# duburcqa/jiminy

Hardware: AMD Instinct MI355X
Metric: env-steps/s (whole node) ANYmal 18-DoF batch 65536; achieved HBM GB/s vs peak (higher is better)
Workload: dtype f64

## Files before the change

jiminy_amd/csrc/jm_quad.h:

```cpp
#pragma once
#include "jm_kernels.h"

namespace jm
{
template<class Tp> struct QLayout
{
    static constexpr int J_PLC = 0, J_RBI = 12, J_AXIS = 22, J_AXP = 25, J_ROTOR = 28, J_QLO = 29, J_QHI = 30, J_MOTOR = 31, J_ENC = 40;
    static constexpr int QJ = 41;
    static constexpr int C_IDX = 12, C_CS = 13, C_FREL = 14;
    static constexpr int QC = Tp::QHAS_FORCE ? 26 : 14;
    static constexpr int CONTACT = Tp::QN * QJ;
    static constexpr int RAW = CONTACT + Tp::QCL * QC;
    static constexpr int QSTRIDE = (RAW % 2 == 0) ? RAW + 1 : RAW;
    static constexpr int TABLE = 4 * QSTRIDE;
    static constexpr int OFFSET = Layout<Tp>::TOTAL;
    static constexpr int TOTAL = OFFSET + TABLE;
};

JM_DEV int sel4(int k, int c0, int c1, int c2, int c3) { return k == 0 ? c0 : (k == 1 ? c1 : (k == 2 ? c2 : c3)); }

template<class Tp> struct QInfo
{
    static constexpr int N = Tp::QN, NT = Tp::QT;
    static constexpr int NQB = 7 + (NT - 1), NVB = 6 + (NT - 1);
    static constexpr bool limb_at(int t)
    {
        for (int k = 0; k < 4; ++k) if (Tp::limb_attach[k] == t) return true;
        return false;
    }
    static constexpr bool child_after(int t, int c)
    {
        for (int i = c + 1; i < NT; ++i) if (Tp::trunk_parent[i] == t) return true;
        return false;
    }
    static constexpr bool has_child(int t) { return limb_at(t) || child_after(t, t); }
    static constexpr bool first_contrib(int c) { return !limb_at(Tp::trunk_parent[c]) && !child_after(Tp::trunk_parent[c], c); }
    static constexpr bool uniform_attach = Tp::limb_attach[0] == Tp::limb_attach[1] && Tp::limb_attach[0] == Tp::limb_attach[2] && Tp::limb_attach[0] == Tp::limb_attach[3];
    static constexpr int qrow(int i) { return i < 7 ? Tp::idx_q[1] + i : Tp::idx_q[Tp::trunk_joint[i - 6]]; }
    static constexpr int vrow(int i) { return i < 6 ? Tp::idx_v[1] + i : Tp::idx_v[Tp::trunk_joint[i - 5]]; }
};

template<class Tp> constexpr int limb_axis_uniform(int s)
{
    int ax = -2;
    for (int k = 0; k < 4; ++k)
    {
        const int c = s < Tp::limb_len[k] ? Tp::axis_signed[Tp::limb_joint[k][s]] : 1;
        if (c == 0) return -1;
        const int a = (c < 0 ? -c : c) - 1;
        if (ax == -2) ax = a;
        else if (ax != a) return -1;
    }
    return ax;
}
template<class Tp> constexpr bool limb_axis_negative(int s)
{
    for (int k = 0; k < 4; ++k)
        if (s < Tp::limb_len[k] && Tp::axis_signed[Tp::limb_joint[k][s]] < 0) return true;
    return false;
}
template<class T> JM_DEV V3<T> mcol(const M3<T> & R, int ax)
{
    return ax == 0 ? V3<T>{R.m00, R.m10, R.m20} : (ax == 1 ? V3<T>{R.m01, R.m11, R.m21} : V3<T>{R.m02, R.m12, R.m22});
}
template<class T> JM_DEV M3<T> mul_rot_axis(const M3<T> & R, int ax, T c, T s)
{
    if (ax == 0) return {R.m00, c * R.m01 + s * R.m02, c * R.m02 - s * R.m01, R.m10, c * R.m11 + s * R.m12, c * R.m12 - s * R.m11,
                         R.m20, c * R.m21 + s * R.m22, c * R.m22 - s * R.m21};
    if (ax == 1) return {c * R.m00 - s * R.m02, R.m01, c * R.m02 + s * R.m00, c * R.m10 - s * R.m12, R.m11, c * R.m12 + s * R.m10,
                         c * R.m20 - s * R.m22, R.m21, c * R.m22 + s * R.m20};
    return {c * R.m00 + s * R.m01, c * R.m01 - s * R.m00, R.m02, c * R.m10 + s * R.m11, c * R.m11 - s * R.m10, R.m12,
            c * R.m20 + s * R.m21, c * R.m21 - s * R.m20, R.m22};
}
template<class T> struct LimbTable
{
    const T * base;
    JM_DEV T operator()(int off) const { return base[off]; }
    JM_DEV V3<T> v3(int o) const { return {base[o], base[o + 1], base[o + 2]}; }
    JM_DEV M3<T> m3(int o) const { return {base[o], base[o + 1], base[o + 2], base[o + 3], base[o + 4], base[o + 5], base[o + 6], base[o + 7], base[o + 8]}; }
    JM_DEV SE3<T> se3(int o) const { return {m3(o), v3(o + 9)}; }
    JM_DEV RBI<T> rbi(int o) const { return {base[o], v3(o + 1), S3<T>{base[o + 4], base[o + 5], base[o + 6], base[o + 7], base[o + 8], base[o + 9]}}; }
};
template<class T, class Tp, int s> JM_DEV V3<T> limb_axis_root(const LimbTable<T> & LT, const M3<T> & Rs_)
{
// ... 456 lines not shown
    {
        a = R * LT.v3(o + Q::J_AXP);
        R = R * (plc.R * rot_rodrigues(LT.v3(o + Q::J_AXIS), c, sn));
    }
}
template<class T, class Tp, int s, class MA = NoModelLane>
JM_DEV void limb_unwind(const LimbTable<T> & LT, T c, T sn, M3<T> & R, V3<T> & p, const MA & ma = MA{}, int k = 0)
{
    using Q = QLayout<Tp>;
    constexpr int o = s * Q::QJ;
    SE3<T> plc = LT.se3(o + Q::J_PLC);
    if constexpr (!std::is_same<MA, NoModelLane>::value)
        plc.p = ma.plc_p(sel4(k, Tp::limb_joint[0][s], Tp::limb_joint[1][s], Tp::limb_joint[2][s], Tp::limb_joint[3][s]), plc.p);
    constexpr int ax = limb_axis_uniform<Tp>(s);
    M3<T> Rq;
    if constexpr (ax >= 0) Rq = mul_rot_axis(R, ax, c, -sn);
    else Rq = R * rot_rodrigues(LT.v3(o + Q::J_AXIS), c, -sn);
    R = mul_bt(Rq, plc.R);
    p = p - R * plc.p;
}

template<class T> JM_DEV Sp<T> applied_wrench_on(const BatchArgs<T> & A, int jq, const M3<T> & R1, const M3<T> & Rj, V3<T> pj,
                                                 unsigned B32, unsigned r32, T te)
{
    Sp<T> f = zero6<T>();
    for (int i = 0; i < A.applied_k; ++i)
    {
        if (A.applied_joint[i] != jq) continue;
        V3<T> F = zero3<T>(), M = zero3<T>();
        if (A.applied)
        {
            const unsigned o = (unsigned)(6 * i) * B32 + r32;
            F = {A.applied[o], A.applied[o + B32], A.applied[o + 2 * B32]};
            M = {A.applied[o + 3 * B32], A.applied[o + 4 * B32], A.applied[o + 5 * B32]};
        }
        if (A.proc_off > 0) add_process_forces(A, i, te, (long long)B32, (long long)r32, F, M);
        const V3<T> p = pj + Rj * V3<T>{A.applied_p[3 * i], A.applied_p[3 * i + 1], A.applied_p[3 * i + 2]};
        const V3<T> fl = tmul(R1, F);
        f.l = f.l + fl;
        f.a = f.a + tmul(R1, M) + cross(p, fl);
    }
    return f;
}
template<class T> JM_DEV Sp<T> applied_root_wrench(const BatchArgs<T> & A, const M3<T> & R1, unsigned B32, unsigned r32, T te)
{
    return applied_wrench_on(A, 1, R1, ident3<T>(), zero3<T>(), B32, r32, te);
}
template<class T> JM_DEV Sp<T> wrench_to_joint(const M3<T> & Rj, V3<T> pj, Sp<T> w)
{
    return {tmul(Rj, w.l), tmul(Rj, w.a - cross(pj, w.l))};
}

template<class T, class Tp> struct QExtra
{
    T tau_l[Tp::QN], tau_b[Tp::QT], uemit_l[Tp::QN], uemit_b[Tp::QT];
    bool motors_on;
    const int32_t * flags;
    const T * lam;
    int nb;
};
struct NoKeep { static constexpr bool ON = false; };
template<class T, class Tp> struct TrunkStore;
template<class T, class Tp> struct QKeep
{
    static constexpr bool ON = true;
    V3<T> ps[Tp::QN], as[Tp::QN];
    Sp<T> Us[Tp::QN];
    T dinv[Tp::QN];
    M3<T> Rt;
    Sp<T> vtip, atip;
    M3<T> R1; V3<T> p1;
    Sp<T> agf1;
    T rootL[6][6], rootdinv[6];
};

template<class T, class Tp, class X, bool EMIT, class SB, int CFM = 0, class KEEP = NoKeep, bool GEN = false, bool DYN = true>
JM_DEV void quad_eval(CPtr<T> P, const LimbTable<T> & LT, const BatchArgs<T> & A, unsigned r, int k, const QIdx<Tp> & ix,
                      const SB & S_, const T * qb, const T * vb_, const T * ql, const T * vl_,
                      bool sensors, T * ddqb, T * ddq, int & status, const QExtra<T, Tp> * ex = nullptr, KEEP * keep = nullptr,
                      TrunkStore<T, Tp> * ts_out = nullptr, T te = T(0))
{
    (void)te;
    using RW = QRows<Tp>;
    auto vlq = [&](int s) -> T { if constexpr (RW::LONG) return S_.getl(RW::KVL + s); else return vl_[s]; };
    auto vbq = [&](int i) -> T { if constexpr (RW::LONG) return S_.getb(RW::KVB + i); else return vb_[i]; };
    auto cmdlq = [&](int s) -> T { return S_.getl(RW::CMDL + s); };
    auto cmdbq = [&](int t) -> T { return S_.getb(RW::CMDB + t); };
    constexpr bool emit = EMIT;
    using L = Layout<Tp>;
    using Q = QLayout<Tp>;
    using I = QInfo<Tp>;
    constexpr int N = Tp::QN, NT = Tp::QT;
    constexpr int FL = Tp::motor_flags[0];
    const unsigned B32 = (unsigned)A.B;
    unsigned r32 = r;
    JM_OPAQUE(r32);
    unsigned Bg = B32, rg = r32;
    if constexpr (GEN)
        if (A.lane_map) { rg = (unsigned)A.lane_map[r32]; Bg = (unsigned)A.B_full; }
    const bool lead = (k == 0);
    const bool emit_sens = emit && sensors;
    const bool want_energy = emit && A.energy;
    if constexpr (Tp::QHAS_ENC)
        if (emit_sens && A.encoder)
        {
            static_for<0, N>([&](auto sc) {
                constexpr int s = decltype(sc)::value;
                const int si = sel4(k, Tp::limb_enc[0][s], Tp::limb_enc[1][s], Tp::limb_enc[2][s], Tp::limb_enc[3][s]);
                T pos = ql[s], vel = vlq(s);
                if constexpr (Tp::QENC_SIDE == 0)
                {
                    const T red = LT(s * Q::QJ + Q::J_ENC);
                    pos *= red;
                    vel *= red;
                }
                if (ix.has[s])
                {
                    A.encoder[(unsigned)(2 * si) * B32 + r32] = pos;
                    A.encoder[(unsigned)(2 * si + 1) * B32 + r32] = vel;
                }
            });
            if (lead)
                static_for<1, NT>([&](auto tc) {
                    constexpr int t = decltype(tc)::value;
                    constexpr int si = Tp::trunk_enc[t];
                    T pos = qb[6 + t], vel = vbq(5 + t);
                    if constexpr (Tp::QENC_SIDE == 0) { pos *= P[L::ENC + si]; vel *= P[L::ENC + si]; }
                    A.encoder[(unsigned)(2 * si) * B32 + r32] = pos;
                    A.encoder[(unsigned)(2 * si + 1) * B32 + r32] = vel;
                });
        }
    const M3<T> R1 = quat_to_matrix(qb[3], qb[4], qb[5], qb[6]);
    const V3<T> p1 = {qb[0], qb[1], qb[2]};
    V3<T> p1g = p1;
    if constexpr (GEN)
        if (A.ground_off) { p1g.x += A.ground_off[rg]; p1g.y += A.ground_off[Bg + rg]; }
    const V3<T> g = ld_v3<T>(P, L::OPT), gw = ld_v3<T>(P, L::OPT + 3);
    const Sp<T> v1 = {{vb_[0], vb_[1], vb_[2]}, {vb_[3], vb_[4], vb_[5]}};
    const Sp<T> agf1 = actinv_motion(SE3<T>{R1, p1}, Sp<T>{-g, -gw});
    TrunkStore<T, Tp> TS;
#ifdef JM_HOST_EMU
    std::memset(&TS, 0xFF, sizeof(TS));
#endif
    SE3<T> Xatt;
    Sp<T> vatt;
    using MA = std::conditional_t<GEN, ModelLane<T>, NoModelLane>;
    MA ma;
    if constexpr (GEN) ma = ModelLane<T>{A.model_lane, Bg, rg};
    auto limb_joint_of = [&](auto sc) {
        constexpr int s = decltype(sc)::value;
        return sel4(k, Tp::limb_joint[0][s], Tp::limb_joint[1][s], Tp::limb_joint[2][s], Tp::limb_joint[3][s]);
    };
    (void)limb_joint_of;
    trunk_fk_store<T, Tp, X, MA>(P, k, ix, qb, vb_, TS, Xatt, vatt, status, ma);
    constexpr bool UNWIND = QRows<Tp>::LONG || !DYN;
    constexpr bool REWIND = UNWIND;
    M3<T> Rs[UNWIND ? 1 : N];
    V3<T> ps[N];
    T cq[UNWIND ? N : 1], sq[UNWIND ? N : 1];
    M3<T> Rtip;
    V3<T> ptip;
    Sp<T> vtip;
    if constexpr (UNWIND) limb_fk_tip<T, Tp, MA>(LT, Xatt, vatt, ql, vl_, cq, sq, Rtip, ptip, vtip, status, ma, k);
    else
    {
        limb_fk<T, Tp, MA>(LT, ix, Xatt, vatt, ql, vl_, Rs, ps, vtip, status, ma, k);
        Rtip = Rs[N - 1]; ptip = ps[N - 1];
    }
// ... 367 lines not shown
                        const Sp<T> vf = actinv_motion(fr, vj);
                        Sp<T> af = actinv_motion(fr, aj);
                        af.l = af.l + cross(vf.a, vf.l);
                        const V3<T> acc3 = af.l - tmul(fr.R, gj);
                        put6(A.imu, B32, r32, 6 * s, Sp<T>{vf.a, acc3});
                    }
                });
    };
    imu_at(std::integral_constant<int, 0>{}, SE3<T>{ident3<T>(), zero3<T>()}, v1r, at0);
    Sp<T> ap = at0;
    Sp<T> vp = v1r;
    M3<T> Rw = ident3<T>();
    V3<T> pw = zero3<T>();
    Sp<T> atst[TrunkStore<T, Tp>::SLOTS];
    {
        Sp<T> aprev = at0;
        static_for<1, NT>([&](auto tc) {
            constexpr int t = decltype(tc)::value;
            constexpr int tp = Tp::trunk_parent[t];
            SE3<T> Xt;
            Sp<T> vt, Ut;
            T di, uj;
            TS.template get_kin<t, X>(Xt, vt);
            if constexpr (DYN) TS.template get_aba<t, X>(Ut, di, uj);
            const Sp<T> S = trunk_S_at<T, Tp, t>(P, Xt);
            const Sp<T> vj = vbq(5 + t) * S;
            Sp<T> apar;
            if constexpr (tp == 0) apar = at0;
            else if constexpr (tp == t - 1) apar = aprev;
            else apar = qbcast<T, X, TrunkStore<T, Tp>::template lane<tp>()>(atst[TrunkStore<T, Tp>::template slot<tp>()]);
            const Sp<T> ag = apar + cross_mm(vt - vj, vj);
            T dd;
            if constexpr (DYN) { dd = di * (uj - dot6(Ut, ag)); ddqb[5 + t] = dd; }
            else dd = ddqb[5 + t];
            const Sp<T> att = ag + dd * S;
            if (TrunkStore<T, Tp>::template first_fwd<t>() || k == TrunkStore<T, Tp>::template lane<t>())
                atst[TrunkStore<T, Tp>::template slot<t>()] = att;
            aprev = att;
            if constexpr (I::limb_at(t))
                if (ix.attach == t)
                {
                    ap = att; vp = vt;
                    if constexpr (REWIND) { Rw = Xt.R; pw = Xt.p; }
                }
            imu_at(tc, Xt, vt, att);
        });
    }
    if constexpr (DYN)
    static_for<0, N>([&](auto sc) {
        constexpr int s = decltype(sc)::value;
        if constexpr (KEEP_SC)
        {
            const Sp<T> ag = ap + cs[s];
            const T dd = ix.has[s] ? dinv[s] * (u[s] - dot6(Us[s], ag)) : T(0);
            ddq[s] = dd;
            ap = ag + dd * Ss[s];
        }
        else
        {
            V3<T> a_s, p_s;
            if constexpr (REWIND)
            {
                limb_rewind<T, Tp, s, MA>(LT, cq[s], sq[s], Rw, pw, a_s, ma, k);
                p_s = pw;
            }
            else { a_s = as[s]; p_s = ps[s]; }
            const Sp<T> S = {cross(p_s, a_s), a_s};
            const Sp<T> vj = vlq(s) * S;
            const Sp<T> ag = ap + cross_mm(vp, vj);
            const T dd = ix.has[s] ? dinv[s] * (u[s] - dot6(Us[s], ag)) : T(0);
            ddq[s] = dd;
            ap = ag + dd * S;
            vp = vp + vj;
        }
    });
    if constexpr (!DYN && EMIT)
    {
        bool applied_out = false;
        if constexpr (GEN) applied_out = A.applied_k > 0 && A.f_external;
        const bool want_rnea = A.joint_forces || A.centroidal;
        if (want_energy || want_rnea || applied_out)
        {
            const bool has_gw = gw.x != T(0) || gw.y != T(0) || gw.z != T(0);
            Sp<T> acur = ap;
            {
                Sp<T> vrun = vp;
                static_for<0, N>([&](auto sc) {
                    constexpr int s = decltype(sc)::value;
                    V3<T> a_s, p_s;
                    if constexpr (REWIND)
                    {
                        limb_rewind<T, Tp, s, MA>(LT, cq[s], sq[s], Rw, pw, a_s, ma, k);
                        p_s = pw;
                    }
                    else { a_s = limb_axis_root<T, Tp, s>(LT, Rs[s]); p_s = ps[s]; }
                    const Sp<T> S = {cross(p_s, a_s), a_s};
                    const Sp<T> vj = vlq(s) * S;
                    acur = acur + cross_mm(vrun, vj) + ddq[s] * S;
                    vrun = vrun + vj;
                });
            }
            Sp<T> hs = zero6<T>(), fjs = zero6<T>(), fxs = fext, Gs = zero6<T>();
            T ms = T(0), ekin = T(0), erot = T(0);
            V3<T> mcs = zero3<T>();
            {
                Sp<T> vcur = vtip;
                M3<T> Rcur = Rtip;
                V3<T> pcur = ptip;
                static_rfor<0, N>([&](auto sc) {
                    constexpr int s = decltype(sc)::value;
                    constexpr int o = s * Q::QJ;
                    if constexpr (!UNWIND) { Rcur = Rs[s]; pcur = ps[s]; }
                    const RBI<T> Y = rbi_placed(Rcur, pcur, ma.rbi(GEN ? limb_joint_of(sc) : 0, LT.rbi(o + Q::J_RBI)));
                    const V3<T> a = limb_axis_root<T, Tp, s>(LT, Rcur);
                    const Sp<T> S = {cross(pcur, a), a};
                    const Sp<T> h = rbi_mul(Y, vcur);
                    hs = hs + h;
                    fjs = fjs + cross_mf(vcur, h) + rbi_mul(Y, acur);
                    if (has_gw) Gs = Gs + rbi_mul(Y, agf1);
                    if constexpr (s == N - 1) fjs = fjs - fext;
                    if constexpr (GEN)
                        if (A.applied_k > 0)
                        {
                            const Sp<T> w = applied_wrench_on(A, limb_joint_of(sc), R1, Rcur, pcur, Bg, rg, te);
                            fjs = fjs - w;
                            fxs = fxs + w;
                            if (applied_out && ix.has[s]) add6(A.f_external, B32, r32, 6u * (unsigned)limb_joint_of(sc), wrench_to_joint(Rcur, pcur, w));
                        }
                    ms += Y.m;
                    mcs = mcs + Y.m * Y.c;
                    ekin += dot6(vcur, h);
                    erot += LT(o + Q::J_ROTOR) * vlq(s) * vlq(s);
                    if (A.joint_forces && ix.has[s])
                        put6(A.joint_forces, B32, r32, 6 * (unsigned)limb_joint_of(sc), actinv_force(SE3<T>{Rcur, pcur}, fjs));
                    const Sp<T> vj = vlq(s) * S;
                    vcur = vcur - vj;
                    acur = acur - cross_mm(vcur, vj) - ddq[s] * S;
                    if constexpr (UNWIND && s > 0) limb_unwind<T, Tp, s, MA>(LT, cq[s], sq[s], Rcur, pcur, ma, k);
                });
            }
            Sp<T> htot = quad_sum6<T, X>(hs), fxtot = quad_sum6<T, X>(fxs), Gtot = zero6<T>();
            if (has_gw) Gtot = quad_sum6<T, X>(Gs);
            T mtot = X::quad_sum(ms);
            V3<T> mctot = {X::quad_sum(mcs.x), X::quad_sum(mcs.y), X::quad_sum(mcs.z)};
            ekin = X::quad_sum(ekin); erot = X::quad_sum(erot);
            Sp<T> fjT[NT];
            static_for<0, NT>([&](auto tc) {
                constexpr int t = decltype(tc)::value;
                if constexpr (I::limb_at(t))
                {
                    if constexpr (I::uniform_attach) fjT[t] = quad_sum6<T, X>(fjs);
                    else fjT[t] = quad_sum6<T, X>(mask6(ix.attach == t, fjs));
                }
                else fjT[t] = zero6<T>();
            });
            static_rfor<0, NT>([&](auto tc) {
                constexpr int t = decltype(tc)::value;
                constexpr int j = Tp::trunk_joint[t];
                SE3<T> Xt = {ident3<T>(), zero3<T>()};
                Sp<T> vt = v1r, att = at0;
                RBI<T> Y = ma.rbi(j, ld_rbi<T>(P, L::JOINT + j * L::JSTRIDE + 12));
                if constexpr (t > 0)
                {
                    TS.template get_kin<t, X>(Xt, vt);
                    att = qbcast<T, X, TrunkStore<T, Tp>::template lane<t>()>(atst[TrunkStore<T, Tp>::template slot<t>()]);
                    Y = rbi_placed(Xt.R, Xt.p, Y);
                }
                const Sp<T> h = rbi_mul(Y, vt);
                htot = htot + h;
                fjT[t] = fjT[t] + cross_mf(vt, h) + rbi_mul(Y, att);
                if (has_gw) Gtot = Gtot + rbi_mul(Y, agf1);
                if constexpr (GEN)
                    if (A.applied_k > 0)
                    {
                        Sp<T> w;
                        if constexpr (t == 0) w = applied_root_wrench(A, R1, Bg, rg, te);
                        else
                        {
                            w = applied_wrench_on(A, j, R1, Xt.R, Xt.p, Bg, rg, te);
                            if (applied_out && lead) put6(A.f_external, B32, r32, 6 * j, wrench_to_joint(Xt.R, Xt.p, w));
                        }
                        fjT[t] = fjT[t] - w;
                        fxtot = fxtot + w;
                    }
                mtot += Y.m;
                mctot = mctot + Y.m * Y.c;
                ekin += dot6(vt, h);
                if constexpr (t > 0) erot += P[L::ROTOR + Tp::idx_v[j]] * vbq(5 + t) * vbq(5 + t);
                if (A.joint_forces && lead)
                {
                    if constexpr (t > 0) put6(A.joint_forces, B32, r32, 6 * j, actinv_force(Xt, fjT[t]));
                    else put6(A.joint_forces, B32, r32, 6 * j, fjT[t]);
                }
                if constexpr (t > 0) fjT[Tp::trunk_parent[t]] = fjT[Tp::trunk_parent[t]] + fjT[t];
            });
            if (lead)
            {
                if (A.joint_forces) put6(A.joint_forces, B32, r32, 0, zero6<T>());
                if (want_energy)
                {
#pragma unroll
                    for (int i = 0; i < 6; ++i) erot += P[L::ROTOR + Tp::idx_v[1] + i] * vb_[i] * vb_[i];
                    A.energy[r32] = T(0.5) * ekin + T(0.5) * erot;
                    A.energy[B32 + r32] = -(dot(R1 * mctot, g) + mtot * dot(p1, g));
                }
                if (A.centroidal)
                {
                    if (!has_gw) Gtot = {mtot * agf1.l, cross(mctot, agf1.l)};
                    const Sp<T> fBtot = fjT[0] + fxtot - Gtot;
                    const SE3<T> M1 = {R1, p1};
                    const V3<T> c1 = rcp_(mtot) * mctot;
                    const V3<T> com0 = R1 * c1 + p1;
                    Sp<T> hg = act_force(M1, htot), dhg = act_force(M1, fBtot);
                    hg.a = hg.a + cross(hg.l, com0);
                    dhg.a = dhg.a + cross(dhg.l, com0);
                    A.centroidal[r32] = com0.x; A.centroidal[B32 + r32] = com0.y; A.centroidal[2 * B32 + r32] = com0.z;
                    put6(A.centroidal, B32, r32, 3, hg);
                    put6(A.centroidal, B32, r32, 9, dhg);
                }
            }
        }
    }
    if constexpr (KEEP::ON)
    {
        keep->atip = ap;
        if (ts_out) *ts_out = TS;
    }
    if constexpr (DYN)
    {
        bool bad = false;
        static_for<0, I::NVB>([&](auto ic) { bad |= (ddqb[decltype(ic)::value] != ddqb[decltype(ic)::value]); });
        static_for<0, N>([&](auto sc) { bad |= ix.has[decltype(sc)::value] && (ddq[decltype(sc)::value] != ddq[decltype(sc)::value]); });
        if (bad) status |= JM_LANE_NAN;
    }
}

template<class T, class Tp, class X, int CFM = 0, bool GEN = false>
JM_DEV void quad_extra_terms(CPtr<T> P, const LimbTable<T> & LT, const BatchArgs<T> & A, unsigned r32, int k, const QIdx<Tp> & ix,
                             const T * qb, const T * vb, const T * ql, const T * vl, const T * ddqb, const T * ddq,
                             const QExtra<T, Tp> * ex = nullptr, T te = T(0))
{
    (void)te;
    using L = Layout<Tp>;
    using Q = QLayout<Tp>;
    using I = QInfo<Tp>;
    constexpr int N = Tp::QN, NT = Tp::QT;
    const unsigned B32 = (unsigned)A.B;
    unsigned Bg = B32, rg = r32;
    if constexpr (GEN)
        if (A.lane_map) { rg = (unsigned)A.lane_map[r32]; Bg = (unsigned)A.B_full; }
    const bool lead = (k == 0);
    const V3<T> g = ld_v3<T>(P, L::OPT), gw = ld_v3<T>(P, L::OPT + 3);
    const M3<T> R1 = quat_to_matrix(qb[3], qb[4], qb[5], qb[6]);
    const V3<T> p1 = {qb[0], qb[1], qb[2]};
    const SE3<T> M1 = {R1, p1};
    V3<T> p1g = p1;
    if constexpr (GEN)
        if (A.ground_off) { p1g.x += A.ground_off[rg]; p1g.y += A.ground_off[Bg + rg]; }
    const Sp<T> agf1 = actinv_motion(M1, Sp<T>{-g, -gw});
    int status = 0;
    using MA = std::conditional_t<GEN, ModelLane<T>, NoModelLane>;
    MA ma;
    if constexpr (GEN) ma = ModelLane<T>{A.model_lane, Bg, rg};
    TrunkKin<T, Tp> K;
    trunk_fk<T, Tp, MA>(P, qb, vb, K, status, ma);
    Sp<T> at[NT];
    at[0] = {{ddqb[0], ddqb[1], ddqb[2]}, {ddqb[3], ddqb[4], ddqb[5]}};
    static_for<1, NT>([&](auto tc) {
        constexpr int t = decltype(tc)::value;
        const Sp<T> S = trunk_S<T, Tp, t>(P, K);
        at[t] = at[Tp::trunk_parent[t]] + cross_mm(K.v[t], vb[5 + t] * S) + ddqb[5 + t] * S;
    });
    M3<T> Rs[N];
    V3<T> ps[N];
    Sp<T> vs[N];
    {
        Sp<T> vtip;
        limb_fk<T, Tp, MA>(LT, ix, pick_attach<T, Tp>(k, K.X), pick_attach<T, Tp>(k, K.v), ql, vl, Rs, ps, vtip, status, ma, k);
        Sp<T> vp = pick_attach<T, Tp>(k, K.v);
        static_for<0, N>([&](auto sc) {
            constexpr int s = decltype(sc)::value;
            const V3<T> a = Rs[s] * LT.v3(s * Q::QJ + Q::J_AXIS);
            vs[s] = {vp.l + vl[s] * cross(ps[s], a), vp.a + vl[s] * a};
            vp = vs[s];
        });
    }
    Sp<T> fext = zero6<T>();
    {
        auto one_contact = [&](int c) {
            const V3<T> pc = Rs[N - 1] * LT.v3(Q::CONTACT + c * Q::QC + 9) + ps[N - 1];
            if constexpr (CFM == 0)
            {
                T depth = p1.z + dot(V3<T>{R1.m20, R1.m21, R1.m22}, pc);
                V3<T> nG = {T(0), T(0), T(1)};
                if constexpr (GEN)
// ... 297 lines not shown
        {
            T dtl = dt;
            JM_OPAQUE(dtl);
            const T bw = dtl * (rk4 ? ((st == 0 || st == 3) ? T(1.0 / 6.0) : T(1.0 / 3.0)) : T(1));
            const T aw = dtl * ((st == 2) ? T(1) : T(0.5));
            T incb[NVB], q0b[NQB], v0b[NVB], incl[N], v0l[N];
            static_for<0, NQB>([&](auto ic) { q0b[decltype(ic)::value] = S.getb(R::Q0B + decltype(ic)::value); });
            static_for<0, NVB>([&](auto ic) {
                constexpr int i = decltype(ic)::value;
                v0b[i] = S.getb(R::V0B + i);
                const T kv = S.getb(R::KVB + i);
                incb[i] = S.getb(R::ACCVB + i) + bw * kv;
                vb[i] = S.getb(R::ACCAB + i) + bw * ddqb[i];
            });
            static_for<0, N>([&](auto sc) {
                constexpr int s = decltype(sc)::value;
                v0l[s] = S.getl(R::V0L + s);
                const T kv = S.getl(R::KVL + s);
                incl[s] = S.getl(R::ACCVL + s) + bw * kv;
                vl[s] = S.getl(R::ACCAL + s) + bw * ddq[s];
                ql[s] = S.getl(R::Q0L + s);
            });
            if (st != 3)
            {
                static_for<0, NVB>([&](auto ic) {
                    constexpr int i = decltype(ic)::value;
                    S.putb(R::ACCVB + i, incb[i]); S.putb(R::ACCAB + i, vb[i]);
                    incb[i] = aw * S.getb(R::KVB + i);
                    vb[i] = v0b[i] + aw * ddqb[i];
                    S.putb(R::KVB + i, vb[i]);
                });
                static_for<0, N>([&](auto sc) {
                    constexpr int s = decltype(sc)::value;
                    S.putl(R::ACCVL + s, incl[s]); S.putl(R::ACCAL + s, vl[s]);
                    incl[s] = aw * S.getl(R::KVL + s);
                    vl[s] = v0l[s] + aw * ddq[s];
                    S.putl(R::KVL + s, vl[s]);
                });
            }
            else
            {
                static_for<0, NVB>([&](auto ic) { vb[decltype(ic)::value] = v0b[decltype(ic)::value] + vb[decltype(ic)::value]; });
                static_for<0, N>([&](auto sc) { vl[decltype(sc)::value] = v0l[decltype(sc)::value] + vl[decltype(sc)::value]; });
            }
            integrate_freeflyer<T>(q0b, incb, qb);
            static_for<1, NT>([&](auto tc) { qb[6 + decltype(tc)::value] = q0b[6 + decltype(tc)::value] + incb[5 + decltype(tc)::value]; });
            static_for<0, N>([&](auto sc) {
                constexpr int s = decltype(sc)::value;
                ql[s] = ql[s] + incl[s];
                if (!ix.has[s]) { ql[s] = T(0); vl[s] = T(0); }
            });
            if (st == 3)
            {
                static_for<0, NQB>([&](auto ic) { S.putb(R::Q0B + decltype(ic)::value, qb[decltype(ic)::value]); });
                static_for<0, NVB>([&](auto ic) {
                    constexpr int i = decltype(ic)::value;
                    S.putb(R::V0B + i, vb[i]); S.putb(R::KVB + i, vb[i]); S.putb(R::ACCVB + i, T(0)); S.putb(R::ACCAB + i, T(0));
                });
                static_for<0, N>([&](auto sc) {
                    constexpr int s = decltype(sc)::value;
                    S.putl(R::Q0L + s, ql[s]); S.putl(R::V0L + s, vl[s]); S.putl(R::KVL + s, vl[s]);
                    S.putl(R::ACCVL + s, T(0)); S.putl(R::ACCAL + s, T(0));
                });
                if (last)
                {
                    if (lead)
                    {
                        static_for<0, NQB>([&](auto ic) { A.q[(unsigned)I::qrow(decltype(ic)::value) * B32 + rr] = qb[decltype(ic)::value]; });
                        static_for<0, NVB>([&](auto ic) { A.v[(unsigned)I::vrow(decltype(ic)::value) * B32 + rr] = vb[decltype(ic)::value]; });
                    }
                    static_for<0, N>([&](auto sc) {
                        constexpr int s = decltype(sc)::value;
                        if (ix.has[s])
                        {
                            A.q[(unsigned)ix.rq[s] * B32 + rr] = ql[s];
                            A.v[(unsigned)ix.rv[s] * B32 + rr] = vl[s];
                        }
                    });
                }
            }
        }
    };
    unsigned rr = r32;
    if constexpr (QCON)
    {
        const int start_passes = INIT == 1 ? 4 : (INIT == 0 ? (A.mode == MODE_REFRESH ? -1 : 0) :
                                 ((A.mode == MODE_START || A.mode == MODE_RESET) ? 4 : (A.mode == MODE_REFRESH ? -1 : 0)));
        if constexpr (PH != 0)
        {
            const int e = split_e;
            const int st = (e < pre) ? -1 : (rk4 ? ((e - pre) & 3) : 3);
            const bool last = e == n_evals - 1;
            if constexpr (PH == 1)
            {
                advance(st, last, rr);
                static_for<0, NQB>([&](auto ic) { S.putb(SR::CURQB + decltype(ic)::value, qb[decltype(ic)::value]); });
                static_for<0, NVB>([&](auto ic) { S.putb(SR::CURVB + decltype(ic)::value, vb[decltype(ic)::value]); });
                static_for<0, N>([&](auto sc) {
                    S.putl(SR::CURQL + decltype(sc)::value, ql[decltype(sc)::value]);
                    S.putl(SR::CURVL + decltype(sc)::value, vl[decltype(sc)::value]);
                });
            }
            quad_eval_con<T, Tp, X, StageBuf<T, SL, SB>, CAPC, GEN, PH, INIT>(P, LT, A, *C, *V, rr, k, ix, S, qb, vb, ql, vl, last,
                                    !stepping || A.update_sensors != 0, ddqb, ddq, status,
                                    INIT == 1 ? 4 : (INIT == 0 ? 0 : ((A.mode == MODE_START || A.mode == MODE_RESET) ? 4 : 0)));
            if (PH == 1 || !last)
            {
                S.putl(SR::STATUSL, (T)status);
                if constexpr (PH == 2)
                {
                    static_for<0, NVB>([&](auto ic) { S.putb(SR::DDQB + decltype(ic)::value, ddqb[decltype(ic)::value]); });
                    static_for<0, N>([&](auto sc) { S.putl(SR::DDQL + decltype(sc)::value, ddq[decltype(sc)::value]); });
                }
                return;
            }
        }
        else
        {
#pragma nounroll
        for (int e = 0; e < n_evals; ++e)
        {
            const int st = (e < pre) ? -1 : (rk4 ? ((e - pre) & 3) : 3);
            const bool last = e == n_evals - 1;
            JM_REFRESH();
            rr = r32;
            JM_OPAQUE(rr);
            advance(st, last, rr);
            if (stepping) stage_time(st);
            quad_eval_con<T, Tp, X, StageBuf<T, SL, SB>, CAPC, GEN, 0, INIT>(P, LT, A, *C, *V, rr, k, ix, S, qb, vb, ql, vl, last && A.mode != MODE_DYNAMICS,
                                    (!stepping && A.mode != MODE_REFRESH) || A.update_sensors != 0, ddqb, ddq, status,
                                    start_passes, te);
        }
        }
    }
    else
    {
    if (stepping)
    {
#pragma nounroll
        for (int e = 0; e < n_evals; ++e)
        {
            const int st = (e < pre) ? -1 : (rk4 ? ((e - pre) & 3) : 3);
            JM_REFRESH();
            rr = r32;
            JM_OPAQUE(rr);
            CPtr<T> Pl = P;
            if constexpr (R::LONG && !GEN) JM_OPAQUE_S(Pl);
            advance(st, e == n_evals - 1, rr);
            stage_time(st);
            quad_eval<T, Tp, X, false, StageBuf<T, SL, SB>, 0, NoKeep, GEN>(Pl, LT, A, rr, k, ix, S, qb, vb, ql, vl, false, ddqb, ddq, status,
                                                                             nullptr, nullptr, nullptr, te);
        }
    }
    else
    {
        JM_REFRESH();
        rr = r32;
        JM_OPAQUE(rr);
        advance(-1, true, rr);
        quad_eval<T, Tp, X, false, StageBuf<T, SL, SB>, 0, NoKeep, GEN>(P, LT, A, rr, k, ix, S, qb, vb, ql, vl, false, ddqb, ddq, status,
                                                                         nullptr, nullptr, nullptr, te);
    }
    if (A.mode != MODE_DYNAMICS)
    {
        JM_REFRESH();
        rr = r32;
        JM_OPAQUE(rr);
        static_for<0, NQB>([&](auto ic) { qb[decltype(ic)::value] = S.getb(R::Q0B + decltype(ic)::value); });
        static_for<0, NVB>([&](auto ic) { vb[decltype(ic)::value] = S.getb(R::V0B + decltype(ic)::value); });
        static_for<0, N>([&](auto sc) { ql[decltype(sc)::value] = S.getl(R::Q0L + decltype(sc)::value); vl[decltype(sc)::value] = S.getl(R::V0L + decltype(sc)::value); });
        quad_eval<T, Tp, X, true, StageBuf<T, SL, SB>, 0, NoKeep, GEN, false>(P, LT, A, rr, k, ix, S, qb, vb, ql, vl,
                                  (!stepping && A.mode != MODE_REFRESH) || A.update_sensors != 0, ddqb, ddq, status,
                                  nullptr, nullptr, nullptr, te);
    }
    }
    {
        T * adst = (A.mode == MODE_DYNAMICS) ? A.a_out : A.a;
        if (lead) static_for<0, NVB>([&](auto ic) { adst[(unsigned)I::vrow(decltype(ic)::value) * B32 + rr] = ddqb[decltype(ic)::value]; });
        static_for<0, N>([&](auto sc) { if (ix.has[decltype(sc)::value]) adst[(unsigned)ix.rv[decltype(sc)::value] * B32 + rr] = ddq[decltype(sc)::value]; });
        if (A.mode != MODE_DYNAMICS)
        {
            const int stq = X::quad_or(status);
            if (A.status && lead) A.status[rr] = (A.mode == MODE_REFRESH) ? (A.status[rr] | stq) : stq;
            if constexpr (GEN && PH == 0)
                if (stepping && lead && A.proc_off > 0) proc_block(A).lane_time()[rr] = tl;
            if constexpr (QCON)
            if (A.joint_forces || A.centroidal)
            {
                JM_REFRESH();
                static_for<0, NQB>([&](auto ic) { qb[decltype(ic)::value] = S.getb(R::Q0B + decltype(ic)::value); });
                static_for<0, NVB>([&](auto ic) { vb[decltype(ic)::value] = S.getb(R::V0B + decltype(ic)::value); });
                static_for<0, N>([&](auto sc) { ql[decltype(sc)::value] = S.getl(R::Q0L + decltype(sc)::value); vl[decltype(sc)::value] = S.getl(R::V0L + decltype(sc)::value); });
                QExtra<T, Tp> ex;
                ex.flags = C->flags;
                ex.nb = qcon_first_contact_row<Tp>();
                ex.lam = C->data + (size_t)qcon_first_lambda_row<Tp>() * B32;
                quad_extra_terms<T, Tp, X, 2, GEN>(P, LT, A, rr, k, ix, qb, vb, ql, vl, ddqb, ddq, &ex, te);
            }
        }
    }
}

#ifndef JM_HOST_EMU
struct DppQuad
{
    template<int CTRL> static __device__ __forceinline__ int mov(int v) { return __builtin_amdgcn_update_dpp(0, v, CTRL, 0xf, 0xf, true); }
    template<int CTRL> static __device__ __forceinline__ double perm(double x)
    {
        const int lo = mov<CTRL>(__double2loint(x)), hi = mov<CTRL>(__double2hiint(x));
        return __hiloint2double(hi, lo);
    }
    template<int CTRL> static __device__ __forceinline__ float perm(float x) { return __int_as_float(mov<CTRL>(__float_as_int(x))); }
    template<int CTRL> static __device__ __forceinline__ int perm(int x) { return mov<CTRL>(x); }
    template<class T> static __device__ __forceinline__ T quad_sum(T x)
    {
        x = x + perm<0xB1>(x);
        x = x + perm<0x4E>(x);
        return x;
    }
    template<int LANE, class T> static __device__ __forceinline__ T bcast(T x) { return perm<LANE * 0x55>(x); }
    static __device__ __forceinline__ int quad_or(int x)
    {
        x |= mov<0xB1>(x);
        x |= mov<0x4E>(x);
        return x;
    }
    template<int CTRL, class T> static __device__ __forceinline__ T perm_(T x) { return perm<CTRL>(x); }
    static __device__ __forceinline__ bool wave_any(bool p) { return __builtin_amdgcn_ballot_w64(p) != 0ull; }
    static __device__ __forceinline__ double max_abs(double a, double b)
    {
        double r;
        asm("v_max_f64 %0, %1, |%2|" : "=v"(r) : "v"(a), "v"(b));
        return r;
    }
    static __device__ __forceinline__ double max_(double a, double b)
    {
        double r;
        asm("v_max_f64 %0, %1, %2" : "=v"(r) : "v"(a), "v"(b));
        return r;
    }
    static __device__ __forceinline__ float max_abs(float a, float b) { return fmaxf(a, fabsf(b)); }
    static __device__ __forceinline__ float max_(float a, float b) { return fmaxf(a, b); }
    static __device__ __forceinline__ void sync() {}
    static __device__ __forceinline__ void fence() { __builtin_amdgcn_fence(__ATOMIC_SEQ_CST, "workgroup"); }
    static __device__ __forceinline__ void table_ready() { __syncthreads(); }
};

template<class T, class Tp> constexpr int quad_block_waves()
{
    constexpr long per_wave = (long)sizeof(T) * (QRows<Tp>::NL * 64 + QRows<Tp>::NB * 16);
    constexpr long table = (long)sizeof(T) * QLayout<Tp>::TABLE;
    int best = 1, best_resident = 0;
    for (int w = 1; w <= 4; w *= 2)
    {
        long blocks = (160L * 1024) / (table + w * per_wave);
        if (blocks * w > 8) blocks = 8 / w;
        const int resident = (int)blocks * w;
        if (resident >= best_resident) { best = w; best_resident = resident; }
    }
    return best;
}
template<class T, class Tp, int W, bool GEN = false> constexpr int quad_waves_per_eu()
{
    constexpr long per_wave = (long)sizeof(T) * (QRows<Tp>::NL * 64 + QRows<Tp>::NB * 16);
    constexpr long block = (long)sizeof(T) * QLayout<Tp>::TABLE + W * per_wave;
    return (!GEN && !QRows<Tp>::LONG && Tp::QT == 1 && Tp::QCL <= 2 && (8 / W) * block <= 160L * 1024) ? 2 : 1;
// ... 38 lines not shown
```

Baseline: 461.0 million.

## Recompute root placement and velocities from stage rows in quad output pass

In the non-dynamics emit pass, base and limb velocities are now read from the staged V0 rows instead of register copies. Root placement, the gravity field and the spatial base velocity/acceleration are recomputed from staged Q0/V0 rows rather than kept live (R1, p1, agf1, v1r, at0). The reverse limb sweep now starts from the forward-sweep end state instead of stored tip/per-limb transforms. The REFRESH status load is issued early with a vmem wait, replacing a refresh barrier. The aim is to cut register pressure and spills in the output pass at the cost of recomputing quaternion-to-matrix transforms and extra scratch reads.

Result: faster. 489.9 million (median of 6 runs) (+6.3%).

```diff
diff --git a/jiminy_amd/csrc/jm_quad.h b/jiminy_amd/csrc/jm_quad.h
--- a/jiminy_amd/csrc/jm_quad.h
+++ b/jiminy_amd/csrc/jm_quad.h
@@ -1,5 +1,13 @@
 #pragma once
 #include "jm_kernels.h"
+
+#ifdef JM_HOST_EMU
+#define JM_OUTPUT_PASS_BEGIN() ((void)0)
+#define JM_WAIT_VMEM() ((void)0)
+#else
+#define JM_OUTPUT_PASS_BEGIN() asm volatile("; quad output pass" ::: "memory")
+#define JM_WAIT_VMEM() __builtin_amdgcn_s_waitcnt(0x0F70)
+#endif
 
 namespace jm
 {
@@ -622,8 +630,17 @@
 {
     (void)te;
     using RW = QRows<Tp>;
-    auto vlq = [&](int s) -> T { if constexpr (RW::LONG) return S_.getl(RW::KVL + s); else return vl_[s]; };
-    auto vbq = [&](int i) -> T { if constexpr (RW::LONG) return S_.getb(RW::KVB + i); else return vb_[i]; };
+    constexpr bool ROWS_V = !DYN && sizeof(T) == 8;
+    auto vlq = [&](int s) -> T {
+        if constexpr (RW::LONG) return S_.getl(RW::KVL + s);
+        else if constexpr (ROWS_V) return S_.getl(RW::V0L + s);
+        else return vl_[s];
+    };
+    auto vbq = [&](int i) -> T {
+        if constexpr (RW::LONG) return S_.getb(RW::KVB + i);
+        else if constexpr (ROWS_V) return S_.getb(RW::V0B + i);
+        else return vb_[i];
+    };
     auto cmdlq = [&](int s) -> T { return S_.getl(RW::CMDL + s); };
     auto cmdbq = [&](int t) -> T { return S_.getb(RW::CMDB + t); };
     constexpr bool emit = EMIT;
@@ -1157,9 +1174,15 @@
         if (want_energy || want_rnea || applied_out)
         {
             const bool has_gw = gw.x != T(0) || gw.y != T(0) || gw.z != T(0);
+            JM_REFRESH();
+            auto root_placement = [&]() -> SE3<T> {
+                return {quat_to_matrix(S_.getb(RW::Q0B + 3), S_.getb(RW::Q0B + 4), S_.getb(RW::Q0B + 5), S_.getb(RW::Q0B + 6)),
+                        V3<T>{S_.getb(RW::Q0B + 0), S_.getb(RW::Q0B + 1), S_.getb(RW::Q0B + 2)}};
+            };
+            auto gravity_field = [&]() -> Sp<T> { return actinv_motion(root_placement(), Sp<T>{-g, -gw}); };
             Sp<T> acur = ap;
-            {
-                Sp<T> vrun = vp;
+            Sp<T> vrun = vp;
+            {
                 static_for<0, N>([&](auto sc) {
                     constexpr int s = decltype(sc)::value;
                     V3<T> a_s, p_s;
@@ -1179,20 +1202,19 @@
             T ms = T(0), ekin = T(0), erot = T(0);
             V3<T> mcs = zero3<T>();
             {
-                Sp<T> vcur = vtip;
-                M3<T> Rcur = Rtip;
-                V3<T> pcur = ptip;
+                Sp<T> vcur = vrun;
+                M3<T> Rcur = Rw;
+                V3<T> pcur = pw;
                 static_rfor<0, N>([&](auto sc) {
                     constexpr int s = decltype(sc)::value;
                     constexpr int o = s * Q::QJ;
-                    if constexpr (!UNWIND) { Rcur = Rs[s]; pcur = ps[s]; }
                     const RBI<T> Y = rbi_placed(Rcur, pcur, ma.rbi(GEN ? limb_joint_of(sc) : 0, LT.rbi(o + Q::J_RBI)));
                     const V3<T> a = limb_axis_root<T, Tp, s>(LT, Rcur);
                     const Sp<T> S = {cross(pcur, a), a};
                     const Sp<T> h = rbi_mul(Y, vcur);
                     hs = hs + h;
                     fjs = fjs + cross_mf(vcur, h) + rbi_mul(Y, acur);
-                    if (has_gw) Gs = Gs + rbi_mul(Y, agf1);
+                    if (has_gw) Gs = Gs + rbi_mul(Y, gravity_field());
                     if constexpr (s == N - 1) fjs = fjs - fext;
                     if constexpr (GEN)
                         if (A.applied_k > 0)
@@ -1219,6 +1241,11 @@
             T mtot = X::quad_sum(ms);
             V3<T> mctot = {X::quad_sum(mcs.x), X::quad_sum(mcs.y), X::quad_sum(mcs.z)};
             ekin = X::quad_sum(ekin); erot = X::quad_sum(erot);
+            const SE3<T> M1 = root_placement();
+            const Sp<T> agf1x = actinv_motion(M1, Sp<T>{-g, -gw});
+            const Sp<T> v1x = {{S_.getb(RW::V0B + 0), S_.getb(RW::V0B + 1), S_.getb(RW::V0B + 2)},
+                               {S_.getb(RW::V0B + 3), S_.getb(RW::V0B + 4), S_.getb(RW::V0B + 5)}};
+            const Sp<T> at0x = agf1x + Sp<T>{{ddqb[0], ddqb[1], ddqb[2]}, {ddqb[3], ddqb[4], ddqb[5]}};
             Sp<T> fjT[NT];
             static_for<0, NT>([&](auto tc) {
                 constexpr int t = decltype(tc)::value;
@@ -1233,7 +1260,7 @@
                 constexpr int t = decltype(tc)::value;
                 constexpr int j = Tp::trunk_joint[t];
                 SE3<T> Xt = {ident3<T>(), zero3<T>()};
-                Sp<T> vt = v1r, att = at0;
+                Sp<T> vt = v1x, att = at0x;
                 RBI<T> Y = ma.rbi(j, ld_rbi<T>(P, L::JOINT + j * L::JSTRIDE + 12));
                 if constexpr (t > 0)
                 {
@@ -1244,15 +1271,15 @@
                 const Sp<T> h = rbi_mul(Y, vt);
                 htot = htot + h;
                 fjT[t] = fjT[t] + cross_mf(vt, h) + rbi_mul(Y, att);
-                if (has_gw) Gtot = Gtot + rbi_mul(Y, agf1);
+                if (has_gw) Gtot = Gtot + rbi_mul(Y, agf1x);
                 if constexpr (GEN)
                     if (A.applied_k > 0)
                     {
                         Sp<T> w;
-                        if constexpr (t == 0) w = applied_root_wrench(A, R1, Bg, rg, te);
+                        if constexpr (t == 0) w = applied_root_wrench(A, M1.R, Bg, rg, te);
                         else
                         {
-                            w = applied_wrench_on(A, j, R1, Xt.R, Xt.p, Bg, rg, te);
+                            w = applied_wrench_on(A, j, M1.R, Xt.R, Xt.p, Bg, rg, te);
                             if (applied_out && lead) put6(A.f_external, B32, r32, 6 * j, wrench_to_joint(Xt.R, Xt.p, w));
                         }
                         fjT[t] = fjT[t] - w;
@@ -1275,17 +1302,16 @@
                 if (want_energy)
                 {
 #pragma unroll
-                    for (int i = 0; i < 6; ++i) erot += P[L::ROTOR + Tp::idx_v[1] + i] * vb_[i] * vb_[i];
+                    for (int i = 0; i < 6; ++i) erot += P[L::ROTOR + Tp::idx_v[1] + i] * S_.getb(RW::V0B + i) * S_.getb(RW::V0B + i);
                     A.energy[r32] = T(0.5) * ekin + T(0.5) * erot;
-                    A.energy[B32 + r32] = -(dot(R1 * mctot, g) + mtot * dot(p1, g));
+                    A.energy[B32 + r32] = -(dot(M1.R * mctot, g) + mtot * dot(M1.p, g));
                 }
                 if (A.centroidal)
                 {
-                    if (!has_gw) Gtot = {mtot * agf1.l, cross(mctot, agf1.l)};
+                    if (!has_gw) Gtot = {mtot * agf1x.l, cross(mctot, agf1x.l)};
                     const Sp<T> fBtot = fjT[0] + fxtot - Gtot;
-                    const SE3<T> M1 = {R1, p1};
                     const V3<T> c1 = rcp_(mtot) * mctot;
-                    const V3<T> com0 = R1 * c1 + p1;
+                    const V3<T> com0 = M1.R * c1 + M1.p;
                     Sp<T> hg = act_force(M1, htot), dhg = act_force(M1, fBtot);
                     hg.a = hg.a + cross(hg.l, com0);
                     dhg.a = dhg.a + cross(dhg.l, com0);
@@ -1749,6 +1775,7 @@
         }
     };
     unsigned rr = r32;
+    int status_before = 0;
     if constexpr (QCON)
     {
         const int start_passes = INIT == 1 ? 4 : (INIT == 0 ? (A.mode == MODE_REFRESH ? -1 : 0) :
@@ -1830,7 +1857,9 @@
     }
     if (A.mode != MODE_DYNAMICS)
     {
-        JM_REFRESH();
+        JM_OUTPUT_PASS_BEGIN();
+        if (A.mode == MODE_REFRESH && A.status && lead) status_before = A.status[r32];
+        JM_WAIT_VMEM();
         rr = r32;
         JM_OPAQUE(rr);
         static_for<0, NQB>([&](auto ic) { qb[decltype(ic)::value] = S.getb(R::Q0B + decltype(ic)::value); });
@@ -1848,7 +1877,8 @@
         if (A.mode != MODE_DYNAMICS)
         {
             const int stq = X::quad_or(status);
-            if (A.status && lead) A.status[rr] = (A.mode == MODE_REFRESH) ? (A.status[rr] | stq) : stq;
+            if constexpr (QCON) { if (A.status && lead) A.status[rr] = (A.mode == MODE_REFRESH) ? (A.status[rr] | stq) : stq; }
+            else if (A.status && lead) A.status[rr] = status_before | stq;
             if constexpr (GEN && PH == 0)
                 if (stepping && lead && A.proc_off > 0) proc_block(A).lane_time()[rr] = tl;
             if constexpr (QCON)
```
